# Vanlightly/vsr-tlaplus

Hardware: NVIDIA H100
Metric: unique states explored/sec (VSR.tla, shipped VSR.cfg constants) (higher is better)
Workload: dtype u32

## Files before the change

vsr-tlaplus_b200/csrc/vsr_actions.h:

```cpp
#ifndef VSR_ACTIONS_H
#define VSR_ACTIONS_H

#include <utility>

#include "vsr_layout.h"

namespace vsr {

struct RunCfg {
    int symmetry;
    int use_view;
    int invariant;
};

template <class L> struct Ops {
    static constexpr int R = L::R, V = L::V, K = L::K, O = L::O;

    static VSR_HD int primary(int v) { return (v - 1) % R; }
    static VSR_HD int oidx(int a, int b) { return b < a ? b : b - 1; }
    static VSR_HD int oinv(int a, int i) { return i < a ? i : i + 1; }

    template <int B, int N = 0, class W> static VSR_HD int loglen(const W& w, int row) {
        int n = 0;
        for (int i = 0; i < V; i++) {
            if (fget<B, L::OB, N>(w, row * V + i) == 0) break;
            n++;
        }
        return n;
    }
    template <int BD, int BS, class WD, class WS> static VSR_HD void logcopy(const WD& wd, int rowd, const WS& ws, int rows) {
        for (int i = 0; i < V; i++) fset<BD, L::OB>(wd, rowd * V + i, fget<BS, L::OB>(ws, rows * V + i));
    }
    template <int B, class W> static VSR_HD void logclear(const W& w, int row) {
        for (int i = 0; i < V; i++) fset<B, L::OB>(w, row * V + i, 0);
    }
    template <class W> static VSR_HD int popmask_svc(const W& w, int r) {
        int n = 0;
        for (int s = 0; s < R; s++) n += (int)VGET(L, SVC_MASK, w, r * R + s);
        return n;
    }
    template <class W> static VSR_HD int popmask_dvc(const W& w, int r) {
        int n = 0;
        for (int s = 0; s < R; s++) n += (int)VGET(L, DVC_MASK, w, r * R + s);
        return n;
    }
    template <class W> static VSR_HD void reset_recv(const W& w, int r) {
        for (int s = 0; s < R; s++) {
            VSET(L, SVC_MASK, w, r * R + s, 0);
            VSET(L, DVC_MASK, w, r * R + s, 0);
        }
        logclear<L::SELF_LOG_B>(w, r);
        VSET(L, SELF_LNV, w, r, 0);
        VSET(L, SELF_COMMIT, w, r, 0);
    }
    template <class W> static VSR_HD void reset_dvc_only(const W& w, int r) {
        for (int s = 0; s < R; s++) VSET(L, DVC_MASK, w, r * R + s, 0);
        logclear<L::SELF_LOG_B>(w, r);
        VSET(L, SELF_LNV, w, r, 0);
        VSET(L, SELF_COMMIT, w, r, 0);
    }
    template <class W> static VSR_HD void reset_sent(const W& w, int r) {
        VSET(L, SENT_DVC, w, r, 0);
        VSET(L, SENT_SV, w, r, 0);
    }
    static VSR_HD int svc_slot(int v, int s, int d) { return ((v - 2) * R + s) * O + oidx(s, d); }
    template <class W> static VSR_HD int broadcast_svc(const W& w, int v, int s) {
        for (int dp = 0; dp < O; dp++) {
            const int idx = ((v - 2) * R + s) * O + dp;
            if (VGET(L, SVC_ST, w, idx) != ST_ABSENT) return E_SLOT_OCCUPIED;
            VSET(L, SVC_ST, w, idx, ST_PENDING);
        }
        return 0;
    }
    template <class W> static VSR_HD int ncreated(const W& w) {
        int c = 0;
        for (int x = 0; x < V; x++) c += VGET(L, PR_VIEW, w, x) != 0;
        return c;
    }

    static constexpr int NGRP = 13;
    static VSR_HD constexpr int grp_begin(int g) {
        const int b[NGRP + 1] = {L::C_TIMER, L::C_HSVC, L::C_SDVC, L::C_HDVC, L::C_SSV, L::C_RSV, L::C_CREQ, L::C_RPREP,
                                 L::C_RPOK, L::C_EXEC, L::C_SGS, L::C_RGS, L::C_RNS, L::NCAND};
        return b[g];
    }
    template <bool APPLY, class S, class N> static VSR_HD int step(const RunCfg& run, const S& s, int cand, const N& n) {
        return cand < L::C_HSVC ? step_grp<APPLY, 0, S, N>(run, s, cand, n) : cand < L::C_SDVC ? step_grp<APPLY, 1, S, N>(run, s, cand, n)
             : cand < L::C_HDVC ? step_grp<APPLY, 2, S, N>(run, s, cand, n) : cand < L::C_SSV ? step_grp<APPLY, 3, S, N>(run, s, cand, n)
             : cand < L::C_RSV ? step_grp<APPLY, 4, S, N>(run, s, cand, n) : cand < L::C_CREQ ? step_grp<APPLY, 5, S, N>(run, s, cand, n)
             : cand < L::C_RPREP ? step_grp<APPLY, 6, S, N>(run, s, cand, n) : cand < L::C_RPOK ? step_grp<APPLY, 7, S, N>(run, s, cand, n)
             : cand < L::C_EXEC ? step_grp<APPLY, 8, S, N>(run, s, cand, n) : cand < L::C_SGS ? step_grp<APPLY, 9, S, N>(run, s, cand, n)
             : cand < L::C_RGS ? step_grp<APPLY, 10, S, N>(run, s, cand, n) : cand < L::C_RNS ? step_grp<APPLY, 11, S, N>(run, s, cand, n)
             : step_grp<APPLY, 12, S, N>(run, s, cand, n);
    }
    template <bool APPLY, int GRP, class S, class N> static VSR_HD int step_grp(const RunCfg& run, const S& s, int cand, const N& n) {
        if constexpr (APPLY) {
            for (int i = 0; i < L::NW; i++) wrw(n, i, rdw(s, i));
        }
        if constexpr (GRP == 0) {
            const int r = cand - L::C_TIMER;
            const int aux = (int)VGET(L, AUX_SVC, s, 0);
            if (!(aux < L::L)) return 0;
            const int v = (int)VGET(L, VIEWN, s, r);
// ... 260 lines not shown
            for (int p = 0; p < R; p++) q += (int)VGET(L, PEER, s, r * R + p) >= cn + 1;
            if (!(q >= R / 2)) return 0;
            if (!APPLY) return 1;
            VSET(L, COMMIT, n, r, cn + 1);
            VSET(L, CT_EXEC, n, r, 1);
            const int x = (int)VGET(L, LOG, s, r * V + cn);
            VSET(L, ACKED, n, x - 1, ACK_TRUE);
            return 1;
        }
        if constexpr (GRP == 10) {
            const int c = cand - L::C_SGS;
            const int j = c % O, dp = (c / O) % O, x = c / (O * O);
            const int pv = (int)VGET(L, PR_VIEW, s, x);
            if (pv == 0) return 0;
            if (VGET(L, PR_CONS, s, x * O + dp)) return 0;
            const int src = primary(pv);
            const int r = oinv(src, dp);
            const int rdest = oinv(r, j);
            const int vr = (int)VGET(L, VIEWN, s, r);
            if (primary(vr) == r) return 0;
            if (VGET(L, STATUS, s, r) != 0) return 0;
            if (!(pv > vr)) return 0;
            const int len = loglen<L::LOG_B, L::LOG_N>(s, r);
            if (!((int)VGET(L, PR_OP, s, x) > len + 1)) return 0;
            const int cn = (int)VGET(L, COMMIT, s, r);
            const int t = cn <= len ? cn : len;
            const int gi = (pv - 2) * O + oidx(src, r);
            if (VGET(L, GS_ST, s, gi) != ST_ABSENT) {
                if ((int)VGET(L, GS_T, s, gi) == t && (int)VGET(L, GS_DEST, s, gi) == rdest) return 0;
                return APPLY ? E_SLOT_OCCUPIED : 1;
            }
            if (!APPLY) return 1;
            if (popmask_svc(s, r) != 0 || popmask_dvc(s, r) != 0) return E_STALE_RECV;
            for (int i = t; i < V; i++) VSET(L, LOG, n, r * V + i, 0);
            VSET(L, VIEWN, n, r, pv);
            VSET(L, LNV, n, r, pv);
            VSET(L, GS_ST, n, gi, ST_PENDING);
            VSET(L, GS_T, n, gi, t);
            VSET(L, GS_DEST, n, gi, rdest);
            return 1;
        }
        if constexpr (GRP == 11) {
            const int gi = cand - L::C_RGS;
            if (VGET(L, GS_ST, s, gi) != ST_PENDING) return 0;
            const int v = gi / O + 2;
            const int r = (int)VGET(L, GS_DEST, s, gi);
            if ((int)VGET(L, VIEWN, s, r) != v) return 0;
            if (VGET(L, STATUS, s, r) != 0) return 0;
            const int t = (int)VGET(L, GS_T, s, gi);
            const int len = loglen<L::LOG_B, L::LOG_N>(s, r);
            if (!(len > t)) return 0;
            if (!APPLY) return 1;
            VSET(L, GS_ST, n, gi, ST_CONSUMED);
            if (VGET(L, NS_ST, s, gi) != ST_ABSENT) return E_SLOT_OCCUPIED;
            VSET(L, NS_ST, n, gi, ST_PENDING);
            for (int i = 0; i < V; i++) VSET(L, NS_LOG, n, gi * V + i, (i >= t && i < len) ? VGET(L, LOG, s, r * V + i) : 0);
            VSET(L, NS_COMMIT, n, gi, VGET(L, COMMIT, s, r));
            return 1;
        }
        if constexpr (GRP == 12) {
            const int gi = cand - L::C_RNS;
            if (VGET(L, NS_ST, s, gi) != ST_PENDING) return 0;
            const int v = gi / O + 2;
            const int r = oinv(primary(v), gi % O);
            if ((int)VGET(L, VIEWN, s, r) != v) return 0;
            if (VGET(L, STATUS, s, r) != 0) return 0;
            const int t = (int)VGET(L, GS_T, s, gi);
            if (loglen<L::LOG_B, L::LOG_N>(s, r) != t) return 0;
            if (!APPLY) return 1;
            for (int i = t; i < V; i++) VSET(L, LOG, n, r * V + i, VGET(L, NS_LOG, s, gi * V + i));
            VSET(L, NS_ST, n, gi, ST_CONSUMED);
            return 1;
        }
        return 0;
    }

    static VSR_HD constexpr int grp_size(int g) { return grp_begin(g + 1) - grp_begin(g); }
    static VSR_HD constexpr int grp_words(int g) { return (grp_size(g) + 31) / 32; }
    template <int G, class S, int... I>
    static VSR_HD void enabled_seq(const RunCfg& run, const S& s, uint32_t* mask, std::integer_sequence<int, I...>) {
        ((mask[I >> 5] |= (uint32_t)(step_grp<false, G>(run, s, grp_begin(G) + I, (uint32_t*)nullptr) > 0) << (I & 31)), ...);
    }
    template <int G, class S> static VSR_HD void enabled_group(const RunCfg& run, const S& s, uint32_t* mask) {
        enabled_seq<G>(run, s, mask, std::make_integer_sequence<int, grp_size(G)>());
    }

    template <int G> static VSR_HD int list_group(const RunCfg& run, const RegRow<L::NW>& st, uint32_t* out, int n) {
        uint32_t m[grp_words(G) > 0 ? grp_words(G) : 1] = {};
        enabled_group<G>(run, st, m);
        for (int i = 0; i < grp_size(G); i++)
            if ((m[i >> 5] >> (i & 31)) & 1u) out[n++] = (uint32_t)(grp_begin(G) + i);
        if constexpr (G + 1 < NGRP) return list_group<G + 1>(run, st, out, n);
        else return n;
    }
    static VSR_HD int enabled_list(const RunCfg& run, const uint32_t* w, uint32_t* out ) {
        RegRow<L::NW> st;
        for (int i = 0; i < L::NW; i++) st.w[i] = w[i];
        return list_group<0>(run, st, out, 0);
    }

    static VSR_HD int action_of(int cand) {
        return cand < L::C_HSVC ? 1 : cand < L::C_MSVC ? 2 : cand < L::C_SDVC ? 3 : cand < L::C_HDVC ? 4
             : cand < L::C_MDVC ? 5 : cand < L::C_SSV ? 6 : cand < L::C_RSV ? 7 : cand < L::C_CREQ ? 8
             : cand < L::C_RPREP ? 9 : cand < L::C_RPOK ? 10 : cand < L::C_EXEC ? 11 : cand < L::C_SGS ? 12
             : cand < L::C_RGS ? 13 : cand < L::C_RNS ? 14 : 15;
    }

    static VSR_HD void init(uint32_t* w) {
        for (int i = 0; i < L::NW; i++) w[i] = 0;
        for (int r = 0; r < R; r++) {
            VSET(L, VIEWN, w, r, 1);
            VSET(L, CT_EXEC, w, r, 1);
        }
    }

    template <class W> static VSR_HD int invariant(const RunCfg& run, const W& w) {
        if (run.invariant & 256) {
            for (int r = 0; r < R; r++)
                if ((int)VGET(L, COMMIT, w, r) == V) return 256;
        }
        if (!(run.invariant & 3)) return 0;
        for (int x = 0; x < V; x++) {
            if (VGET(L, ACKED, w, x) != ACK_TRUE) continue;
            int holders = 0;
            for (int r = 0; r < R; r++) {
                int has = 0;
                for (int i = 0; i < V; i++) has |= (int)VGET(L, LOG, w, r * V + i) == x + 1;
                holders += has;
            }
            if ((run.invariant & 1) && holders == 0) return 1;
            if ((run.invariant & 2) && holders < R / 2 + 1) return 2;
        }
        return 0;
    }

    template <class W> static VSR_HD bool all_same_view_normal(const RunCfg&, const W& w) {
        const uint32_t v0 = VGET(L, VIEWN, w, 0);
        for (int r = 0; r < R; r++)
            if (VGET(L, STATUS, w, r) != 0 || VGET(L, VIEWN, w, r) != v0) return false;
        return true;
    }
    template <class W> static VSR_HD bool some_commit(const W& w) {
        for (int r = 0; r < R; r++)
            if (VGET(L, COMMIT, w, r) >= 1) return true;
        return false;
    }
    template <class W> static VSR_HD bool live_pred(const RunCfg& run, const W& w, int live_hooks) {
        return (live_hooks & 1) ? some_commit(w) : all_same_view_normal(run, w);
    }

    template <class W> static VSR_HD uint32_t aux_key(const W& w) {
        uint32_t k = VGET(L, AUX_SVC, w, 0);
        k = k * 16u;
        for (int x = 0; x < V; x++) k = k * 3u + VGET(L, ACKED, w, x);
        return k;
    }

    static VSR_HD int literal_cand(const uint32_t* w, int cand) {
        if (cand < L::C_CREQ || cand >= L::C_RGS || (cand >= L::C_RPOK && cand < L::C_SGS)) return cand;
        if (cand < L::C_RPREP) {
            const int r = (cand - L::C_CREQ) / V;
            for (int x = 0; x < V; x++)
                if (VGET(L, PR_VIEW, w, x) == 0) return L::C_CREQ + r * V + x;
            return -1;
        }
        int order[V > 0 ? V : 1], nc = 0;
        for (int x = 0; x < V; x++)
// ... 177 lines not shown
```

vsr-tlaplus_b200/csrc/vsr_gpu.cu:

```cuda
#include <stddef.h>
#include <stdio.h>
#include <stdlib.h>
#include <string.h>

#include <algorithm>
#include <chrono>
#include <string>
#include <vector>

#include "vsr_engine.h"

namespace vsr {

const GpuOps* find_gpu_ops(int R, int V, int K) {
#define X(r, v, k) \
    if (R == r && V == v && K == k) return GpuThunks<Layout<r, v, k>>::get();
    VSR_FOR_EACH_CONFIG(X)
#undef X
    return nullptr;
}

}

using namespace vsr;
// ... 284 lines not shown
int vsr_engine_expand_part(VsrEngine* e, uint64_t first, uint64_t count) { return vsr_engine_step(e, first, count, 0, nullptr, nullptr); }

int vsr_engine_expand(VsrEngine* e) { return vsr_engine_step(e, 0, e->n_cur, 0, nullptr, nullptr); }

int vsr_engine_insert_records(VsrEngine* e, const void* dev_records, uint64_t n) {
    if (!e->level_open) {
        int rc = engine_reset_level(e);
        if (rc) return rc;
    }
    if (n == 0) return 0;
    const int rc = insert_records(e, dev_records, n);
    if (rc) return rc;
    CK(cudaEventSynchronize(e->ev1));
    float ms = 0;
    cudaEventElapsedTime(&ms, e->ev0, e->ev1);
    e->level_ms_acc += ms;
    e->level_ms_insert_acc += ms;
    return 0;
}

int vsr_engine_finish_level(VsrEngine* e, VsrLevelInfo* out) {
    LevelCounters lc;
    DevCounters& c = lc.c;
    const size_t ctr_bytes = e->cov ? sizeof lc : sizeof c;
    CK(cudaMemcpyAsync(&lc, e->ctr, ctr_bytes, cudaMemcpyDeviceToHost, e->stream));
    e->st.bytes_d2h += ctr_bytes;
    CK(cudaStreamSynchronize(e->stream));
    const uint64_t fcap_total = e->frontier_cap + e->frontier_host_cap;
    if (c.tie_count > 0 && c.tie_count <= e->tie_cap && !c.overflow && c.out_count <= fcap_total) {
        const size_t tb = (size_t)e->g->tie_bytes;
        std::vector<uint8_t> host(c.tie_count * tb);
        CK(cudaMemcpyAsync(host.data(), e->ties, host.size(), cudaMemcpyDeviceToHost, e->stream));
        CK(cudaStreamSynchronize(e->stream));
        std::vector<const uint8_t*> recs;
        for (uint64_t i = 0; i < c.tie_count; i++) recs.push_back(host.data() + i * tb);
        auto key = [](const uint8_t* r) { return (const TieRec*)r; };
        std::sort(recs.begin(), recs.end(), [&](const uint8_t* a, const uint8_t* b) {
            const TieRec *x = key(a), *y = key(b);
            if (x->fp != y->fp) return x->fp < y->fp;
            if (x->check != y->check) return x->check < y->check;
            if (x->auxkey != y->auxkey) return x->auxkey < y->auxkey;
            if (x->parent != y->parent) return x->parent < y->parent;
            return x->cand < y->cand;
        });
        std::vector<uint8_t> best;
        uint64_t nbest = 0;
        for (size_t i = 0; i < recs.size(); i++) {
            if (i && key(recs[i])->fp == key(recs[i - 1])->fp && key(recs[i])->check == key(recs[i - 1])->check) continue;
            best.insert(best.end(), recs[i], recs[i] + tb);
            nbest++;
        }
        CK(cudaMemcpyAsync(e->ties, best.data(), best.size(), cudaMemcpyHostToDevice, e->stream));
        static const unsigned long long ones = ~0ull;
        CK(cudaMemcpyAsync(&e->ctr->viol_id, &ones, 8, cudaMemcpyHostToDevice, e->stream));
        CK(cudaMemsetAsync(&e->ctr->viol_which, 0, sizeof(int), e->stream));
        ExpandParams p;
        fill_params(e, p);
        CK(e->g->launch_patch(p, e->ties, nbest, c.out_count, e->stream));
        e->st.kernel_launches++;
        CK(cudaMemcpyAsync(&lc, e->ctr, ctr_bytes, cudaMemcpyDeviceToHost, e->stream));
        CK(cudaStreamSynchronize(e->stream));
        e->st.bytes_d2h += host.size() + ctr_bytes;
        e->st.bytes_h2d += best.size();
    }
    VsrLevelInfo li;
    memset(&li, 0, sizeof li);
    li.new_states = c.out_count;
    li.generated = c.generated;
    li.frontier_in = e->n_cur;
    li.ties = c.ties;
    li.collisions = c.collisions;
    li.violation = c.viol_id != ~0ull;
    li.violation_id = c.viol_id;
    li.violation_mask = c.viol_which;
    li.deadlock = c.dead_id != ~0ull;
    li.deadlock_id = c.dead_id;
    li.error_code = c.error;
    li.overflow = c.overflow;
    li.ms = e->level_ms_acc;
    li.ms_insert = e->level_ms_insert_acc;
#ifdef VSR_EXP_ROUNDCLK
    {
        double all = 0;
        for (int i = 0; i < 5; i++) all += (double)c.roundclk[i];
        if (all > 0)
            fprintf(stderr, "roundclk rank %d depth %d  ms %.4f  warp-Gcycles %.4f  end_barrier %.4f  scan_barriers %.4f  batches %.4f  scan %.4f  other %.4f\n",
                    e->rank, e->level, e->level_ms_acc, all * 1e-9, c.roundclk[0] / all, c.roundclk[1] / all, c.roundclk[2] / all, c.roundclk[3] / all, c.roundclk[4] / all);
    }
#endif
    if (c.overflow) {
        snprintf(e->last_error, sizeof e->last_error, "capacity exceeded (%s): %llu new states this level, frontier capacity %llu",
                 c.overflow == 1 ? "frontier" : (c.overflow == 2 ? "tie list" : (c.overflow == 3 ? "send buffer" : "seen-set")), (unsigned long long)c.out_count,
                 (unsigned long long)fcap_total);
    }
    if (!li.overflow && e->st.distinct + c.out_count > e->table_cap - e->table_cap / 8) {
        li.overflow = 4;
        snprintf(e->last_error, sizeof e->last_error, "capacity exceeded (seen-set): %llu distinct states in %llu slots",
                 (unsigned long long)(e->st.distinct + c.out_count), (unsigned long long)e->table_cap);
    }
    const uint64_t n_new = c.out_count <= fcap_total ? c.out_count : fcap_total;
    e->st.generated += c.generated;
    e->st.distinct += n_new;
    e->st.h2_ties += c.ties;
    e->st.fp_collisions += c.collisions;
    e->st.probe_total += c.probes;
    e->st.seconds_kernels += e->level_ms_acc * 1e-3;
    if (c.error && !e->st.error_code) e->st.error_code = c.error;
    const int gen_level = e->level + 1;
    if (e->level >= 1 && e->level - 1 < VSR_MAX_LEVELS) {
        e->st.level_generated[e->level - 1] = c.generated;
        e->st.level_ms[e->level - 1] = e->level_ms_acc;
        e->st.levels_expanded = e->level;
    }
    if (n_new > 0 && gen_level - 1 < VSR_MAX_LEVELS) {
        e->st.level_sizes[gen_level - 1] = n_new;
        e->st.num_levels = gen_level;
    }
    if (e->cov && gen_level - 1 < VSR_MAX_LEVELS) {
        bool any = false;
        for (int a = 0; a < VSR_NUM_ACTIONS; a++) {
            const uint64_t g = lc.cover[a], d = lc.cover[VSR_NUM_ACTIONS + a];
            e->cov->level_generated[gen_level - 1][a] = g;
            e->cov->level_distinct[gen_level - 1][a] = d;
            e->cov->generated[a] += g;
            e->cov->distinct[a] += d;
            any |= g != 0;
        }
        if (any) e->cov->num_levels = gen_level;
    }
    if (li.violation && e->st.violation_level == 0) {
        e->st.violation_level = gen_level;
        e->st.violation_id = c.viol_id;
    }
    e->cur ^= 1;
    e->cur_base = e->next_base;
    e->n_cur = n_new;
    e->next_base += n_new;
    e->level = gen_level;
    e->level_open = false;
    if (e->live_index && !li.overflow) {
        const int rc = live_collect(e);
        if (rc == VSR_RC_TOO_LARGE) li.overflow = 5;
        else if (rc) return rc;
    }
    if (e->opts.collect_levels) {
        std::vector<uint8_t> host((size_t)n_new * e->g->bytes);
        if (n_new && vsr_engine_read_frontier(e, 0, n_new, host.data())) return VSR_RC_SYSTEM;
        e->collected.push_back(std::move(host));
    }
    if (out) *out = li;
    return 0;
}

uint64_t vsr_engine_frontier_size(const VsrEngine* e) { return e->n_cur; }

int vsr_engine_read_frontier(VsrEngine* e, uint64_t first, uint64_t n, void* host_out) {
    if (first + n > e->n_cur) return VSR_RC_ERROR;
    const uint64_t S = (uint64_t)e->g->bytes;
    const uint64_t in_dev = first < e->frontier_cap ? std::min(n, e->frontier_cap - first) : 0;
    if (in_dev) CK(cudaMemcpy(host_out, (const uint8_t*)e->frontier[e->cur] + first * S, in_dev * S, cudaMemcpyDeviceToHost));
    if (n > in_dev) memcpy((uint8_t*)host_out + in_dev * S, (const uint8_t*)e->frontier_host[e->cur] + (first + in_dev - e->frontier_cap) * S, (n - in_dev) * S);
    return 0;
}

int vsr_engine_trace_record(VsrEngine* e, uint64_t local_id, uint64_t* parent_out, uint32_t* cand_out) {
    if (!e->trace || local_id >= e->trace_cap) return VSR_RC_ERROR;
    uint64_t t = 0;
    CK(cudaMemcpy(&t, e->trace + local_id, 8, cudaMemcpyDeviceToHost));
    e->st.bytes_d2h += 8;
    *parent_out = (t >> 12) & GID_MASK;
// ... 230 lines not shown
```

vsr-tlaplus_b200/csrc/vsr_gpu.cuh:

```cuda
#ifndef VSR_GPU_CUH
#define VSR_GPU_CUH

#include <cuda_runtime.h>
#include <stdint.h>

#include "../../include/vsr_flat.h"
#include "vsr_actions.h"

namespace vsr {

struct DevCounters {
    unsigned long long out_count;
    unsigned long long generated;
    unsigned long long ties;
    unsigned long long collisions;
    unsigned long long probes;
    unsigned long long viol_id;
    unsigned long long dead_id;
    unsigned long long tie_count;
    int error;
    int overflow;
    int viol_which;
    int _pad;
    unsigned long long work_next;
    unsigned long long drain_next;
    unsigned int send_count[8];
#ifdef VSR_EXP_ROUNDCLK
    unsigned long long roundclk[5];
#endif
};
struct LevelCounters {
    DevCounters c;
    unsigned long long cover[2 * VSR_NUM_ACTIONS];
};
#ifdef VSR_EXP_ROUNDCLK
enum { CLK_END = 0, CLK_SCANBAR = 1, CLK_BATCH = 2, CLK_SCAN = 3, CLK_OTHER = 4 };
#endif

struct TieRec {
    uint64_t fp;
    uint64_t parent;
    uint32_t auxkey, cand, check, _pad;
};

struct RecHdr {
    uint64_t fp;
    uint64_t tm;
};
constexpr int MAX_WORLD = 8;


struct ExpandParams {
    const uint32_t* in;
    unsigned long long n_in;
    unsigned long long in_base;
    const uint32_t* in_hi;
    unsigned long long in_split;
    uint32_t* out;
    uint32_t* out_hi;
    unsigned long long out_split;
    unsigned long long out_cap;
    unsigned long long out_base;
    uint64_t* table;
    unsigned long long table_cap;
    uint64_t* trace;
    unsigned long long trace_cap;
    DevCounters* ctr;
    uint8_t* ties;
    unsigned long long tie_cap;
    const uint64_t* fp_tab;
    RunCfg run;
    int level;
    int check_deadlock;
    int rank, world, owner_shift;
    uint8_t* push[MAX_WORLD];
    unsigned long long push_cap;
    const uint8_t* drain[MAX_WORLD];
    unsigned int drain_n[MAX_WORLD];
    unsigned long long drain_total;
    unsigned long long* cover;
};


__device__ __forceinline__ void cas128(uint64_t* p, uint64_t s0, uint64_t s1, uint64_t& o0, uint64_t& o1) {
    asm volatile(
        "{\n\t.reg .b128 cmp, swp, old;\n\tmov.b128 cmp, {%2, %3};\n\tmov.b128 swp, {%4, %5};\n\t"
        "atom.global.relaxed.gpu.cas.b128 old, [%6], cmp, swp;\n\tmov.b128 {%0, %1}, old;\n\t}"
        : "=l"(o0), "=l"(o1)
        : "l"(0ull), "l"(0ull), "l"(s0), "l"(s1), "l"(p)
        : "memory");
}
__device__ __forceinline__ void ld128_cg(const uint64_t* p, uint64_t& a, uint64_t& b) {
    asm volatile("ld.global.cg.v2.u64 {%0, %1}, [%2];" : "=l"(a), "=l"(b) : "l"(p) : "memory");
}
__device__ __forceinline__ uint64_t mix64(uint64_t x) {
    x ^= x >> 30; x *= 0xbf58476d1ce4e5b9ULL;
    x ^= x >> 27; x *= 0x94d049bb133111ebULL;
    x ^= x >> 31;
    return x;
}
template <class L, bool USE_VIEW, class W> VSR_HD uint32_t check_hash_t(const W& w) {
    constexpr int full = L::VIEW_BITS >> 5, rem = L::VIEW_BITS & 31;
    constexpr int nw = USE_VIEW ? (full + (rem ? 1 : 0)) : L::NW;
    uint32_t h = 0x9747b28cu;
VSR_UNROLL
    for (int i = 0; i < nw; i++) {
        uint32_t k = rdw(w, i);
        if (USE_VIEW && i == full) k &= (1u << rem) - 1u;
        h ^= k;
        h = ((h << 13) | (h >> 19)) * 5u + 0xe6546b64u;
    }
    h ^= h >> 16; h *= 0x85ebca6bu; h ^= h >> 13; h *= 0xc2b2ae35u; h ^= h >> 16;
    return h;
}
template <class L, class W> VSR_HD uint32_t check_hash(const W& w, bool use_view) {
    return use_view ? check_hash_t<L, true>(w) : check_hash_t<L, false>(w);
}

enum { INS_NEW = 0, INS_DUP = 1, INS_TIE = 2, INS_FULL = 3 };

constexpr unsigned long long GID_MASK = (1ull << 44) - 1ull, ROOT_GID = GID_MASK;
__host__ __device__ __forceinline__ uint64_t make_gid(int rank, unsigned long long local_id) { return ((uint64_t)rank << 40) | local_id; }
__host__ __device__ __forceinline__ uint64_t make_trec(uint64_t parent_gid, uint32_t cand) { return (parent_gid << 12) | (cand & 0xFFFu); }

__device__ __forceinline__ uint64_t make_meta(int level, uint32_t auxkey, uint32_t check) {
    return ((uint64_t)(uint32_t)level << 56) | ((uint64_t)(auxkey & 0xFFFFFFu) << 32) | check;
}

#ifndef VSR_BUCKET
#define VSR_BUCKET 2
#endif
struct Probe { uint64_t e[2 * VSR_BUCKET]; };
__device__ __forceinline__ void ld256_cg(const uint64_t* p, uint64_t& a, uint64_t& b, uint64_t& c, uint64_t& d) {
    asm volatile("ld.global.cg.v2.u64 {%0, %1}, [%4];\n\tld.global.cg.v2.u64 {%2, %3}, [%4+16];"
                 : "=l"(a), "=l"(b), "=l"(c), "=l"(d) : "l"(p) : "memory");
}
__device__ __forceinline__ unsigned long long table_home(unsigned long long cap, uint64_t fp) {
    return __umul64hi(fp * 0x9E3779B97F4A7C15ULL, cap / VSR_BUCKET) * VSR_BUCKET;
}
__device__ __forceinline__ void probe_load(const uint64_t* table, unsigned long long h, Probe& p) {
#if VSR_BUCKET == 1
    ld128_cg(table + 2 * h, p.e[0], p.e[1]);
#elif VSR_BUCKET == 2
    ld128_cg(table + 2 * h, p.e[0], p.e[1]);
#elif VSR_BUCKET == 4
    ld256_cg(table + 2 * h, p.e[0], p.e[1], p.e[2], p.e[3]);
    ld256_cg(table + 2 * h + 4, p.e[4], p.e[5], p.e[6], p.e[7]);
#else
#error "VSR_BUCKET must be 1, 2 or 4"
#endif
}
__device__ __forceinline__ int table_insert_from(uint64_t* table, unsigned long long cap, unsigned long long h, Probe p, uint64_t fp, uint64_t meta,
                                                 unsigned& probes, unsigned& collisions) {
    for (unsigned tries = 0;; tries++) {
        if (tries > (1u << 16)) return INS_FULL;
        probes++;
VSR_UNROLL
        for (int j = 0; j < VSR_BUCKET; j++) {
            uint64_t e0, e1;
            if (VSR_BUCKET == 2 && j == 1) {
                ld128_cg(table + 2 * (h + 1), e0, e1);
            } else {
                e0 = p.e[2 * j];
                e1 = p.e[2 * j + 1];
            }
            if (e0 == 0) {
                cas128(table + 2 * (h + j), fp, meta, e0, e1);
                if (e0 == 0 && e1 == 0) return INS_NEW;
            }
            for (int again = 0; e1 == 0 && again < 64; again++) ld128_cg(table + 2 * (h + j), e0, e1);
            if (e0 == fp) {
                if ((uint32_t)e1 == (uint32_t)meta) {
                    const bool same_level = (e1 >> 56) == (meta >> 56);
                    const bool same_aux = ((e1 >> 32) & 0xFFFFFF) == ((meta >> 32) & 0xFFFFFF);
// ... 19 lines not shown
    asm volatile("fence.proxy.async.shared::cta;" ::: "memory");
    const uint32_t s = (uint32_t)__cvta_generic_to_shared(ssrc);
    asm volatile("cp.async.bulk.global.shared::cta.bulk_group [%0], [%1], %2;" ::"l"(gdst), "r"(s), "r"(bytes) : "memory");
    asm volatile("cp.async.bulk.commit_group;" ::: "memory");
    asm volatile("cp.async.bulk.wait_group.read 0;" ::: "memory");
}

template <int NW> __device__ __forceinline__ uint32_t* out_state(const ExpandParams& P, unsigned long long i) {
    return i < P.out_split ? P.out + i * NW : P.out_hi + (i - P.out_split) * NW;
}


#ifdef VSR_QPS
constexpr int QPS = VSR_QPS;
#else
constexpr int QPS = 10;
#endif

template <class L, int ROWS> struct WarpStage {
    alignas(16) uint32_t stage[ROWS * L::NW + 32];
    unsigned long long tstage[ROWS];
    int sn;
};
template <class L, int WARPS, int PASSES> struct BlockSmemT {
    typedef WarpStage<L, PASSES == 2 ? 32 : 64> Stage;
    static constexpr int NS = WARPS * 32;
    static constexpr int NR = PASSES * NS;
    static constexpr int NG = 13;
    uint64_t fp_tab[8 * 256];
    uint32_t par[NR * (L::NW + 1)];
    static constexpr int QCAP = QPS * NS;
    uint16_t pool[PASSES * QCAP];
    int qcount[PASSES][NG];
    int take;
    unsigned long long round_first;
    Stage w[WARPS];
};
template <class L> struct ExpandCfg {
    static constexpr size_t SMEM_ONE = 227 * 1024 - 512, SMEM_TWO = 113 * 1024;
    static constexpr int max_grp() { int m = 0; for (int g = 0; g < Ops<L>::NGRP; g++) m = Ops<L>::grp_size(g) > m ? Ops<L>::grp_size(g) : m; return m; }
    template <int W> static constexpr int pick_one() {
        if constexpr (W < 18) return 0;
        else if constexpr (sizeof(BlockSmemT<L, W, 1>) <= SMEM_ONE) return W;
        else return pick_one<W - 2>();
    }
    static constexpr int W2 = sizeof(BlockSmemT<L, 16, 1>) <= SMEM_TWO ? 16 : (sizeof(BlockSmemT<L, 12, 1>) <= SMEM_TWO ? 12 : 8);
    static constexpr int W1 = max_grp() < 64 ? pick_one<32>() : 0;
#ifdef VSR_FORCE_WARPS
    static constexpr int WARPS = VSR_FORCE_WARPS;
#else
    static constexpr int WARPS = W1 >= 2 * W2 - 4 ? W1 : W2;
#endif
    static constexpr int BLOCKS = WARPS > 16 ? 1 : 2;
#ifdef VSR_ROUND_PASSES
    static constexpr int PASSES = VSR_ROUND_PASSES;
#else
    static constexpr int PASSES = BLOCKS == 1 && sizeof(BlockSmemT<L, WARPS, 2>) <= SMEM_ONE ? 2 : 1;
#endif
    typedef BlockSmemT<L, WARPS, PASSES> Smem;
};

template <class L, bool MULTI, bool COVER = false> struct Expander {
    typedef Ops<L> O_;
    typedef typename ExpandCfg<L>::Smem Smem;
    typedef typename Smem::Stage Stage;
    static constexpr int WARPS = ExpandCfg<L>::WARPS, NS = Smem::NS, PASSES = ExpandCfg<L>::PASSES;
    static constexpr int SROWS = PASSES == 2 ? 32 : 64;
    const ExpandParams& P;
    Smem& B;
    Stage& S;
    const int lane, warp, tid;
    const uint32_t* mine = nullptr;
    bool have = false;
    int pass = 0;
    __device__ __forceinline__ int pass_i() const { return PASSES == 1 ? 0 : pass; }

    __device__ Expander(const ExpandParams& p, Smem& b) : P(p), B(b), S(b.w[threadIdx.x >> 5]), lane(threadIdx.x & 31), warp(threadIdx.x >> 5), tid(threadIdx.x) {
#ifdef VSR_EXP_ROUNDCLK
        clk_t = clock64();
#endif
    }

#ifdef VSR_EXP_ROUNDCLK
    unsigned long long clk_t = 0, clk[5] = {};
    __device__ __forceinline__ void clk_mark(int i) {
        const unsigned long long t = clock64();
        clk[i] += t - clk_t;
        clk_t = t;
    }
#define VSR_CLK(X, i) (X).clk_mark(CLK_##i)
#else
#define VSR_CLK(X, i) ((void)0)
#endif

    static __device__ __noinline__ void flush(const ExpandParams& P, Stage& S, int lane, int n) {
        const int sn = SROWS == 32 ? n : S.sn;
        unsigned long long base = 0;
        if (lane == 0) base = atomicAdd(&P.ctr->out_count, (unsigned long long)n);
        base = __shfl_sync(0xffffffffu, base, 0);
        if (lane < n) {
            const unsigned long long t = S.tstage[lane];
            if (t >> 63) {
                atomicMin(&P.ctr->viol_id, P.out_base + base + lane);
                S.tstage[lane] = t & ~(1ull << 63);
            }
        }
        __syncwarp();
        if (base + n > P.out_cap) {
            if (lane == 0) atomicExch(&P.ctr->overflow, 1);
        } else {
            if (lane == 0) {
                if (base + n <= P.out_split) bulk_store(P.out + base * L::NW, S.stage, (uint32_t)(n * L::BYTES));
                else if (base >= P.out_split) bulk_store(P.out_hi + (base - P.out_split) * L::NW, S.stage, (uint32_t)(n * L::BYTES));
                else {
                    const int n1 = (int)(P.out_split - base);
                    bulk_store(P.out + base * L::NW, S.stage, (uint32_t)(n1 * L::BYTES));
                    bulk_store(P.out_hi, S.stage + n1 * L::NW, (uint32_t)((n - n1) * L::BYTES));
                }
            }
            if (P.trace && lane < n && P.out_base + base + lane < P.trace_cap) P.trace[P.out_base + base + lane] = S.tstage[lane];
        }
        __syncwarp();
        const int rest = sn - n;
        for (int i0 = 0; i0 < rest * L::NW; i0 += 32) {
            const int i = i0 + lane;
            uint32_t v = 0;
            if (i < rest * L::NW) v = S.stage[n * L::NW + i];
            __syncwarp();
            if (i < rest * L::NW) S.stage[i] = v;
        }
        unsigned long long t = 0;
        if (lane < rest) t = S.tstage[n + lane];
        __syncwarp();
        if (lane < rest) S.tstage[lane] = t;
        if (lane == 0) S.sn = rest;
        __syncwarp();
    }

    typedef uint32_t* Row;
    static constexpr int gcd32(int a) { int g = 32; while (a % g) g >>= 1; return g; }
    static constexpr int SKEW_P = 32 / gcd32(L::NW);
    static __device__ __forceinline__ Row scratch(Stage& S, int lane) { return &S.stage[(SROWS - 32 + lane) * L::NW + lane / SKEW_P]; }

    static __device__ __forceinline__ void push_records(const ExpandParams& P, Stage& S, int lane, const RegRow<L::NW>& v, int send_to, uint64_t fp,
                                                        uint64_t tm) {
        const unsigned senders = __ballot_sync(0xffffffffu, send_to >= 0);
        if (!senders) return;
        constexpr int RB = L::BYTES + (int)sizeof(RecHdr), RW = RB / 4;
        constexpr int CAPREC = (32 * L::BYTES) / RB;
        static_assert(CAPREC >= 16, "two passes must cover a batch");
        int off = 0, cnt = 0, rnk = 0;
        unsigned mymask = 0;
        for (int d = 0; d < P.world; d++) {
            const unsigned m = __ballot_sync(0xffffffffu, send_to == d);
            if (send_to > d) off += __popc(m);
            if (send_to == d) { mymask = m; cnt = __popc(m); rnk = __popc(m & ((1u << lane) - 1u)); }
        }
        unsigned base = 0;
        if (send_to >= 0 && rnk == 0) base = atomicAdd(&P.ctr->send_count[send_to], (unsigned)cnt);
        base = __shfl_sync(0xffffffffu, base, mymask ? __ffs(mymask) - 1 : 0);
        const bool fits = send_to >= 0 && (unsigned long long)base + (unsigned)cnt <= P.push_cap;
        if (send_to >= 0 && !fits && rnk == 0) atomicExch(&P.ctr->overflow, 3);
        const int pos = off + rnk, total = __popc(senders);
        uint32_t* sbuf = &S.stage[(SROWS - 32) * L::NW];
        for (int lo = 0; lo < total; lo += CAPREC) {
            const int hi = lo + CAPREC < total ? lo + CAPREC : total;
            if (send_to >= 0 && pos >= lo && pos < hi) {
// ... 183 lines not shown
                v.w[4 * q] = x.x; v.w[4 * q + 1] = x.y; v.w[4 * q + 2] = x.z; v.w[4 * q + 3] = x.w;
            }
            chk = check_hash<L>(v, P.run.use_view != 0);
            auxkey = O_::aux_key(v);
        }
        tally(commit(P, S, lane, v, d.have, d.fp, chk, auxkey, d.home, d.first, d.tm & ((1ull << 56) - 1ull), (unsigned)((d.tm >> 56) & 0xFu)));
    }
    __device__ void drain() {
        const unsigned long long nchunks = drain_chunks();
        if (dchunk == ~0ull) dchunk = __shfl_sync(0xffffffffu, drain_claim(), 0);
        while (dchunk < nchunks) {
            const unsigned long long nx = drain_claim();
            const DrainPre d = drain_begin(dchunk);
            drain_end(d);
            dchunk = __shfl_sync(0xffffffffu, nx, 0);
        }
    }

    static constexpr int NG = O_::NGRP;
    static __host__ __device__ constexpr int moff(int g) { int o = 0; for (int h = 0; h < g; h++) o += O_::grp_words(h); return o; }
    static constexpr int MW = moff(NG);
    static constexpr int PW = (NG + 1) / 2;
    static __host__ __device__ constexpr int max_grp() { int m = 0; for (int g = 0; g < NG; g++) m = O_::grp_size(g) > m ? O_::grp_size(g) : m; return m; }
    static constexpr int TBITS = NS <= 512 ? 9 : 10;
    static_assert(NS <= (1 << TBITS) && max_grp() < (1 << (16 - TBITS)), "pool item does not fit 16 bits");
    static_assert(max_grp() * NS < 65536, "16-bit packed counters");

    template <int G> __device__ __forceinline__ void guards(const RegRow<L::NW>& st, uint32_t* m, uint32_t* pc) {
        O_::template enabled_group<G>(P.run, st, m + moff(G));
        uint32_t c = 0;
        VSR_UNROLL
        for (int k = 0; k < O_::grp_words(G); k++) c += (uint32_t)__popc(m[moff(G) + k]);
        pc[G >> 1] += c << (16 * (G & 1));
        if constexpr (G + 1 < NG) guards<G + 1>(st, m, pc);
    }
    template <int G, bool FAST> __device__ __forceinline__ void push(uint32_t* m, const uint32_t* ex, const uint32_t* wb, int st) {
        int pos = st + (int)((wb[G >> 1] >> (16 * (G & 1))) & 0xFFFFu) + (int)((ex[G >> 1] >> (16 * (G & 1))) & 0xFFFFu);
        VSR_UNROLL
        for (int k = 0; k < O_::grp_words(G); k++) {
            uint32_t mm = m[moff(G) + k], left = 0;
            while (mm) {
                const int bit = __ffs(mm) - 1;
                mm &= mm - 1;
                if (FAST || pos < Smem::QCAP) B.pool[pass_i() * Smem::QCAP + pos] = (uint16_t)(tid | ((k * 32 + bit) << TBITS));
                else left |= 1u << bit;
                pos++;
            }
            if (!FAST) m[moff(G) + k] = left;
        }
        if constexpr (G + 1 < NG) {
            const int q = B.qcount[pass_i()][G];
            const int nst = FAST ? st + q : (st + q < Smem::QCAP ? st + q : Smem::QCAP);
            push<G + 1, FAST>(m, ex, wb, nst);
        }
    }
    template <int G> __device__ __forceinline__ void leftovers(uint32_t* m) {
        VSR_UNROLL
        for (int k = 0; k < O_::grp_words(G); k++) {
            while (__any_sync(0xffffffffu, m[moff(G) + k] != 0)) {
                const bool inl = m[moff(G) + k] != 0;
                int cand = 0;
                if (inl) {
                    const int bit = __ffs(m[moff(G) + k]) - 1;
                    m[moff(G) + k] &= m[moff(G) + k] - 1;
                    cand = O_::grp_begin(G) + k * 32 + bit;
                }
                tally(apply<G>(P, B, S, lane, mine, cand, pass_i() * NS + tid, inl));
            }
        }
        if constexpr (G + 1 < NG) leftovers<G + 1>(m);
    }
    __device__ __forceinline__ void scan_all() {
        uint32_t m[MW], pc[PW];
        VSR_UNROLL
        for (int i = 0; i < MW; i++) m[i] = 0;
        VSR_UNROLL
        for (int i = 0; i < PW; i++) pc[i] = 0;
        if (have) {
            RegRow<L::NW> st;
            VSR_UNROLL
            for (int i = 0; i < L::NW; i++) st.w[i] = mine[i];
            guards<0>(st, m, pc);
        }
        uint32_t ex[PW], wb[PW];
        VSR_UNROLL
        for (int i = 0; i < PW; i++) ex[i] = pc[i];
        VSR_UNROLL
        for (int o = 1; o < 32; o <<= 1) {
            VSR_UNROLL
            for (int i = 0; i < PW; i++) {
                const uint32_t t = __shfl_up_sync(0xffffffffu, ex[i], o);
                if (lane >= o) ex[i] += t;
            }
        }
        uint32_t mytot = 0, anyc = 0;
        VSR_UNROLL
        for (int g = 0; g < NG; g++) {
            const uint32_t t = (__shfl_sync(0xffffffffu, ex[g >> 1], 31) >> (16 * (g & 1))) & 0xFFFFu;
            if (lane == g) mytot = t;
        }
        VSR_UNROLL
        for (int i = 0; i < PW; i++) { anyc |= pc[i]; ex[i] -= pc[i]; }
        uint32_t mybase = 0;
        if (lane < NG && mytot) mybase = (uint32_t)atomicAdd(&B.qcount[pass_i()][lane], (int)mytot);
        VSR_UNROLL
        for (int i = 0; i < PW; i++) wb[i] = 0;
        VSR_UNROLL
        for (int g = 0; g < NG; g++) wb[g >> 1] |= (__shfl_sync(0xffffffffu, mybase, g) & 0xFFFFu) << (16 * (g & 1));
        if (P.check_deadlock && have && !anyc) atomicMin(&P.ctr->dead_id, P.in_base + B.round_first + pass_i() * NS + tid);
        VSR_CLK(*this, SCAN);
        __syncthreads();
        VSR_CLK(*this, SCANBAR);
#ifndef VSR_EXP_NO_PUSHFAST
        int all = 0;
        VSR_UNROLL
        for (int g = 0; g < NG; g++) all += B.qcount[pass_i()][g];
        if (all <= Smem::QCAP) {
            push<0, true>(m, ex, wb, 0);
            return;
        }
#endif
        push<0, false>(m, ex, wb, 0);
        uint32_t rest = 0;
        VSR_UNROLL
        for (int i = 0; i < MW; i++) rest |= m[i];
        if (__any_sync(0xffffffffu, rest != 0)) leftovers<0>(m);
    }
    template <int G> static __device__ __noinline__ unsigned long long apply(const ExpandParams& P, Smem& B, Stage& S, int lane,
                                                                             const uint32_t* parent, int cand, int si, bool act) {
        const Row n = scratch(S, lane);
        int mult = 0;
        if (act) mult = O_::template step_grp<true, G>(P.run, parent, cand, n);
        return emit(P, B, S, lane, n, mult, cand, si, act);
    }
    template <int G> static __device__ __forceinline__ unsigned long long batch(const ExpandParams& P, Smem& B, Stage& S, int lane, int b,
                                                                                int k) {
        const bool act = lane < k;
        int cand = 0, si = 0;
        if (act) {
            const unsigned item = B.pool[b + lane];
            si = (PASSES == 1 ? 0 : b / Smem::QCAP) * NS + (int)(item & ((1 << TBITS) - 1));
            cand = O_::grp_begin(G) + (int)(item >> TBITS);
        }
        return apply<G>(P, B, S, lane, &B.par[si * (L::NW + 1)], cand, si, act);
    }
    unsigned long long acc_gen = 0, acc_probes = 0;
    __device__ __forceinline__ void tally(unsigned long long r) {
        acc_gen += (unsigned)r;
        acc_probes += r >> 32;
    }

    __device__ void run_round(unsigned long long first, int count) {
        const uint32_t* src = P.in + first * L::NW;
        if (first + count <= P.in_split) {
            for (int i = tid; i < count * L::NW; i += NS) B.par[(i / L::NW) * (L::NW + 1) + (i % L::NW)] = __ldg(src + i);
        } else {
            for (int i = tid; i < count * L::NW; i += NS) {
                const unsigned long long st = first + i / L::NW;
                const uint32_t* row = st < P.in_split ? P.in + st * L::NW : P.in_hi + (st - P.in_split) * L::NW;
                B.par[(i / L::NW) * (L::NW + 1) + (i % L::NW)] = __ldg(row + i % L::NW);
            }
        }
        if (tid < PASSES * Smem::NG) (&B.qcount[0][0])[tid] = 0;
        if (tid == 0) { B.round_first = first; B.take = 0; }
        VSR_CLK(*this, SCAN);
        __syncthreads();
        VSR_CLK(*this, SCANBAR);
#pragma unroll 1
        for (pass = 0; pass < PASSES; pass++) {
            have = pass_i() * NS + tid < count;
            mine = &B.par[(have ? pass_i() * NS + tid : 0) * (L::NW + 1)];
            scan_all();
        }
        VSR_CLK(*this, SCAN);
        __syncthreads();
        VSR_CLK(*this, SCANBAR);
        static_assert(PASSES * Smem::NG <= 32, "one lane per segment");
        const int sp = lane / Smem::NG;
        const int q = lane < PASSES * Smem::NG ? (&B.qcount[0][0])[lane] : 0;
        int inc = q;
        VSR_UNROLL
        for (int o = 1; o < 32; o <<= 1) {
            const int t = __shfl_up_sync(0xffffffffu, inc, o);
            if (lane >= o) inc += t;
        }
        const int before = __shfl_sync(0xffffffffu, inc, sp * Smem::NG - 1 + (sp == 0));
        if (sp > 0) inc -= before;
        const int seg_st = sp * Smem::QCAP + (inc - q < Smem::QCAP ? inc - q : Smem::QCAP), seg_en = sp * Smem::QCAP + (inc < Smem::QCAP ? inc : Smem::QCAP);
        const int nb = (seg_en - seg_st + 31) >> 5;
        int binc = nb;
        VSR_UNROLL
        for (int o = 1; o < 32; o <<= 1) {
            const int t = __shfl_up_sync(0xffffffffu, binc, o);
            if (lane >= o) binc += t;
        }
        const int total = __shfl_sync(0xffffffffu, binc, 31);
        for (;;) {
            int t = 0;
            if (lane == 0) t = atomicAdd(&B.take, 1);
            t = __shfl_sync(0xffffffffu, t, 0);
            if (t >= total) break;
            const int s = __popc(__ballot_sync(0xffffffffu, lane < PASSES * Smem::NG && binc <= t));
            const int st = __shfl_sync(0xffffffffu, seg_st, s), en = __shfl_sync(0xffffffffu, seg_en, s);
            const int b = st + (t - __shfl_sync(0xffffffffu, binc - nb, s)) * 32;
            const int k = en - b < 32 ? en - b : 32;
            unsigned long long r;
            switch (s % Smem::NG) {
            case 0: r = batch<0>(P, B, S, lane, b, k); break;   case 1: r = batch<1>(P, B, S, lane, b, k); break;
            case 2: r = batch<2>(P, B, S, lane, b, k); break;   case 3: r = batch<3>(P, B, S, lane, b, k); break;
            case 4: r = batch<4>(P, B, S, lane, b, k); break;   case 5: r = batch<5>(P, B, S, lane, b, k); break;
            case 6: r = batch<6>(P, B, S, lane, b, k); break;   case 7: r = batch<7>(P, B, S, lane, b, k); break;
            case 8: r = batch<8>(P, B, S, lane, b, k); break;   case 9: r = batch<9>(P, B, S, lane, b, k); break;
            case 10: r = batch<10>(P, B, S, lane, b, k); break; case 11: r = batch<11>(P, B, S, lane, b, k); break;
            default: r = batch<12>(P, B, S, lane, b, k); break;
            }
            tally(r);
            VSR_CLK(*this, BATCH);
        }
        VSR_CLK(*this, BATCH);
    }

    __device__ void finish() {
        while (S.sn > 0) flush(P, S, lane, S.sn < 32 ? S.sn : 32);
#ifdef VSR_EXP_ROUNDCLK
        clk_mark(CLK_OTHER);
        VSR_UNROLL
        for (int i = 0; i < 5; i++)
            if (lane == 0) atomicAdd(&P.ctr->roundclk[i], clk[i]);
#endif
        for (int o = 16; o; o >>= 1) {
            acc_gen += __shfl_xor_sync(0xffffffffu, acc_gen, o);
            acc_probes += __shfl_xor_sync(0xffffffffu, acc_probes, o);
        }
        if (lane == 0) {
            atomicAdd(&P.ctr->generated, acc_gen);
            atomicAdd(&P.ctr->probes, acc_probes);
        }
        if constexpr (COVER && COVER_SHARED) {
            __syncthreads();
            const unsigned long long* tab = cover_table(P);
            if (tid < NCOV && tab[tid]) atomicAdd(&P.cover[tid], tab[tid]);
        }
    }
};

template <class L, bool MULTI, bool COVER = false> __global__ void __launch_bounds__(ExpandCfg<L>::WARPS * 32, ExpandCfg<L>::BLOCKS) expand_kernel(const __grid_constant__ ExpandParams P) {
    extern __shared__ __align__(128) unsigned char smem_raw[];
    typedef typename ExpandCfg<L>::Smem Smem;
    Smem& B = *reinterpret_cast<Smem*>(smem_raw);
    for (int i = threadIdx.x; i < 8 * 256; i += blockDim.x) B.fp_tab[i] = P.fp_tab[i];
    __shared__ unsigned long long next_round;
    Expander<L, MULTI, COVER> X(P, B);
    if ((threadIdx.x & 31) == 0) B.w[threadIdx.x >> 5].sn = 0;
    if constexpr (COVER && Expander<L, MULTI, COVER>::COVER_SHARED) {
        if (threadIdx.x < Expander<L, MULTI, COVER>::NCOV) Expander<L, MULTI, COVER>::cover_table(P)[threadIdx.x] = 0;
    }
    const unsigned long long nrounds = (P.n_in + Smem::NR - 1) / Smem::NR;
    if (threadIdx.x == 0) next_round = atomicAdd(&P.ctr->work_next, 1ull);
    VSR_CLK(X, OTHER);
    for (;;) {
        __syncthreads();
        const unsigned long long c = next_round;
        __syncthreads();
        VSR_CLK(X, END);
        if (c >= nrounds) break;
        if (threadIdx.x == 0) {
            next_round = atomicAdd(&P.ctr->work_next, 1ull);
            const unsigned long long nx = next_round;
            if (nx < nrounds && (nx + 1) * Smem::NR <= P.in_split) {
                const unsigned long long nfirst = nx * Smem::NR;
                const unsigned long long ncount = (P.n_in - nfirst) < (unsigned long long)Smem::NR ? (P.n_in - nfirst) : Smem::NR;
                asm volatile("cp.async.bulk.prefetch.L2.global [%0], %1;" ::"l"(P.in + nfirst * L::NW), "r"((uint32_t)(ncount * L::BYTES)) : "memory");
            }
        }
        const unsigned long long first = c * Smem::NR;
        const int count = (int)((P.n_in - first) < (unsigned long long)Smem::NR ? (P.n_in - first) : Smem::NR);
        X.run_round(first, count);
    }
    if (MULTI && P.drain_total) X.drain();
    X.finish();
}

template <class L> __global__ void patch_ties_kernel(const ExpandParams P, const uint8_t* ties, unsigned long long ntie, unsigned long long n_out) {
    const unsigned long long i = (unsigned long long)blockIdx.x * blockDim.x + threadIdx.x;
    if (i >= n_out) return;
    uint32_t w[L::NW];
    uint32_t* st = out_state<L::NW>(P, i);
    for (int j = 0; j < L::NW; j++) w[j] = st[j];
    uint64_t fp = fp64_view8<L>(P.fp_tab, w, P.run.use_view != 0);
    if (fp == 0) fp = 1;
    const uint32_t chk = check_hash<L>(w, P.run.use_view != 0);
    const size_t stride = sizeof(TieRec) + L::BYTES;
    unsigned long long lo = 0, hi = ntie;
    while (lo < hi) {
        const unsigned long long mid = (lo + hi) / 2;
        if (((const TieRec*)(ties + mid * stride))->fp < fp) lo = mid + 1; else hi = mid;
    }
    for (; lo < ntie; lo++) {
        const TieRec* t = (const TieRec*)(ties + lo * stride);
        if (t->fp != fp) break;
        if (t->check != chk) continue;
        if (t->auxkey < Ops<L>::aux_key(w)) {
            const uint32_t* tw = (const uint32_t*)((const uint8_t*)t + sizeof(TieRec));
            for (int j = 0; j < L::NW; j++) { w[j] = tw[j]; st[j] = tw[j]; }
            if (P.trace && P.out_base + i < P.trace_cap) {
                if (P.cover) {
                    const uint64_t was = P.trace[P.out_base + i];
                    const int a0 = (was >> 12) == ROOT_GID ? (int)VSR_ACT_INIT : Ops<L>::action_of((int)(was & 0xFFFu));
                    const int a1 = t->parent == ROOT_GID ? (int)VSR_ACT_INIT : Ops<L>::action_of((int)(t->cand & 0xFFFu));
                    if (a0 != a1) {
// ... 221 lines not shown
```

Baseline: 2.969 billion.

## Vectorize guard scans over slot bitmasks and load parent rows with cp.async

Replaces per-candidate guard evaluation for several action groups with word-level bitmask computation. Pending message slots are masked against per-class enable predicates evaluated once per class, and the even bits are compacted into the enabled mask. Groups 11 and 12 now iterate only over pending slots. Parent-state loads into shared memory use cp.async instead of register round-trips, and the clock-profiling buckets are split for finer scan timing. The risk is heavy template code whose slot-to-candidate mapping must exactly match the original per-candidate guards.

After: 3.046 billion (median of 6 runs). +2.6%, better.

```diff
diff --git a/vsr-tlaplus_b200/csrc/vsr_actions.h b/vsr-tlaplus_b200/csrc/vsr_actions.h
--- a/vsr-tlaplus_b200/csrc/vsr_actions.h
+++ b/vsr-tlaplus_b200/csrc/vsr_actions.h
@@ -16,9 +16,9 @@
 template <class L> struct Ops {
     static constexpr int R = L::R, V = L::V, K = L::K, O = L::O;
 
-    static VSR_HD int primary(int v) { return (v - 1) % R; }
-    static VSR_HD int oidx(int a, int b) { return b < a ? b : b - 1; }
-    static VSR_HD int oinv(int a, int i) { return i < a ? i : i + 1; }
+    static VSR_HD constexpr int primary(int v) { return (v - 1) % R; }
+    static VSR_HD constexpr int oidx(int a, int b) { return b < a ? b : b - 1; }
+    static VSR_HD constexpr int oinv(int a, int i) { return i < a ? i : i + 1; }
 
     template <int B, int N = 0, class W> static VSR_HD int loglen(const W& w, int row) {
         int n = 0;
@@ -445,7 +445,112 @@
         ((mask[I >> 5] |= (uint32_t)(step_grp<false, G>(run, s, grp_begin(G) + I, (uint32_t*)nullptr) > 0) << (I & 31)), ...);
     }
     template <int G, class S> static VSR_HD void enabled_group(const RunCfg& run, const S& s, uint32_t* mask) {
+#ifndef VSR_EXP_SCAN_PERCAND
+        if constexpr (G == 1 || G == 3 || G == 5 || G == 8) {
+            enabled_slots<G>(run, s, mask);
+            return;
+        } else if constexpr (G == 11 || G == 12) {
+            enabled_pending<G>(run, s, mask);
+            return;
+        }
+#endif
         enabled_seq<G>(run, s, mask, std::make_integer_sequence<int, grp_size(G)>());
+    }
+
+    static VSR_HD constexpr int slot_cls(int g, int i) {
+        return g == 1 ? (i / (O * R)) * R + oinv((i / O) % R, i % O)
+             : g == 3 ? i / O
+             : g == 5 ? (i / O) * R + oinv(primary(i / O + 2), i % O)
+             : i;
+    }
+    static VSR_HD constexpr int slot_base(int g) { return g == 1 ? L::SVC_ST_B : g == 3 ? L::DVC_ST_B : g == 5 ? L::SV_ST_B : g == 8 ? L::POK_ST_B : g == 11 ? L::GS_ST_B : L::NS_ST_B; }
+    static VSR_HD constexpr int slot_n(int g) { return g == 1 ? L::NSVC : g == 3 ? L::NDVC : g == 5 ? L::NSV : g == 8 ? L::NPOK : L::NGS; }
+    static VSR_HD constexpr int slot_ncls(int g) { return g == 1 ? L::NV2 * R : g == 3 ? L::NV2 : g == 5 ? L::NV2 * R : slot_n(g); }
+    static VSR_HD constexpr int slot_outs(int g) { return g == 1 || g == 3 ? 2 : 1; }
+    static VSR_HD constexpr uint32_t cls_mask(int g, int k, int c) {
+        uint32_t m = 0;
+        for (int i = 0; i < slot_n(g); i++) {
+            const int p = slot_base(g) + 2 * i;
+            if ((p >> 5) == k && (c < 0 || slot_cls(g, i) == c)) m |= 1u << (p & 31);
+        }
+        return m;
+    }
+    template <int G, int K, int C> static constexpr uint32_t CLS_MASK = cls_mask(G, K, C);
+    template <int G, int OUT, int C, class S> static VSR_HD bool cls_on(const S& s) {
+        if constexpr (G == 1) {
+            constexpr int v = C / R + 2, r = C % R;
+            const int vr = (int)VGET(L, VIEWN, s, r);
+            if constexpr (OUT == 0) return v > vr;
+            else return v == vr && VGET(L, STATUS, s, r) == 1;
+        } else if constexpr (G == 3) {
+            constexpr int v = C + 2, r = primary(v);
+            const int vr = (int)VGET(L, VIEWN, s, r);
+            return OUT == 0 ? v > vr : v == vr;
+        } else if constexpr (G == 5) {
+            constexpr int v = C / R + 2, r = C % R;
+            return v >= (int)VGET(L, VIEWN, s, r);
+        } else {
+            constexpr int sp = C % O, nn = (C / O) % V + 1, v = C / (O * V) + 1;
+            constexpr int r = primary(v), src = oinv(r, sp);
+            return v == (int)VGET(L, VIEWN, s, r) && VGET(L, STATUS, s, r) == 0 && nn > (int)VGET(L, PEER, s, r * R + src);
+        }
+    }
+    template <int G, int OUT, int K, class S, int... C> static VSR_HD uint32_t sel_word(const S& s, std::integer_sequence<int, C...>) {
+        uint32_t m = 0;
+        ((m |= (CLS_MASK<G, K, C> != 0u && cls_on<G, OUT, C>(s)) ? CLS_MASK<G, K, C> : 0u), ...);
+        return m;
+    }
+    static VSR_HD uint32_t gather_even(uint32_t x) {
+        x &= 0x55555555u;
+        x = (x | (x >> 1)) & 0x33333333u;
+        x = (x | (x >> 2)) & 0x0F0F0F0Fu;
+        x = (x | (x >> 4)) & 0x00FF00FFu;
+        return (x | (x >> 8)) & 0x0000FFFFu;
+    }
+    template <int G, int SH> static VSR_HD void put_bits(uint32_t* mask, uint32_t c) {
+        if constexpr (SH < 0) {
+            put_bits<G, 0>(mask, c >> -SH);
+        } else {
+            mask[SH >> 5] |= c << (SH & 31);
+            if constexpr ((SH & 31) > 16 && (SH >> 5) + 1 < grp_words(G)) mask[(SH >> 5) + 1] |= c >> (32 - (SH & 31));
+        }
+    }
+    template <int G, int K, class S> static VSR_HD uint32_t pending_word(const S& s) {
+        const uint32_t w = rdw(s, K);
+        return w & ~(w >> 1) & CLS_MASK<G, K, -1>;
+    }
+    template <int G, int K, class S> static VSR_HD void slots_word(const S& s, uint32_t* mask) {
+        constexpr int B = slot_base(G), N = slot_n(G);
+        const uint32_t pend = pending_word<G, K>(s);
+        constexpr int D = 16 * K - B / 2;
+        put_bits<G, D>(mask, gather_even(pend & sel_word<G, 0, K>(s, std::make_integer_sequence<int, slot_ncls(G)>())));
+        if constexpr (slot_outs(G) == 2) put_bits<G, D + N>(mask, gather_even(pend & sel_word<G, 1, K>(s, std::make_integer_sequence<int, slot_ncls(G)>())));
+        if constexpr (K + 1 <= ((B + 2 * N - 1) >> 5)) slots_word<G, K + 1>(s, mask);
+    }
+    template <int G, class S> static VSR_HD void enabled_slots(const RunCfg&, const S& s, uint32_t* mask) {
+        static_assert(slot_base(G) % 2 == 0, "2-bit slots start at even bits");
+        if constexpr (slot_n(G) > 0) slots_word<G, (slot_base(G) >> 5)>(s, mask);
+    }
+    template <int G, int K, class S> static VSR_HD void pending_loop(const RunCfg& run, const S& s, uint32_t* mask) {
+        constexpr int B = slot_base(G);
+        uint32_t pend = pending_word<G, K>(s);
+        while (pend) {
+#if defined(__CUDA_ARCH__)
+            const int bit = __ffs(pend) - 1;
+#else
+            const int bit = __builtin_ctz(pend);
+#endif
+            pend &= pend - 1;
+            const int i = (32 * K + bit - B) >> 1;
+            if (step_grp<false, G>(run, s, grp_begin(G) + i, (uint32_t*)nullptr) > 0) {
+                VSR_UNROLL
+                for (int q = 0; q < grp_words(G); q++) mask[q] |= (i >> 5) == q ? 1u << (i & 31) : 0u;
+            }
+        }
+        if constexpr (K + 1 <= ((B + 2 * slot_n(G) - 1) >> 5)) pending_loop<G, K + 1>(run, s, mask);
+    }
+    template <int G, class S> static VSR_HD void enabled_pending(const RunCfg& run, const S& s, uint32_t* mask) {
+        if constexpr (slot_n(G) > 0) pending_loop<G, (slot_base(G) >> 5)>(run, s, mask);
     }
 
     template <int G> static VSR_HD int list_group(const RunCfg& run, const RegRow<L::NW>& st, uint32_t* out, int n) {
diff --git a/vsr-tlaplus_b200/csrc/vsr_gpu.cu b/vsr-tlaplus_b200/csrc/vsr_gpu.cu
--- a/vsr-tlaplus_b200/csrc/vsr_gpu.cu
+++ b/vsr-tlaplus_b200/csrc/vsr_gpu.cu
@@ -390,10 +390,13 @@
 #ifdef VSR_EXP_ROUNDCLK
     {
         double all = 0;
-        for (int i = 0; i < 5; i++) all += (double)c.roundclk[i];
+        for (int i = 0; i < CLK_N; i++) all += (double)c.roundclk[i];
         if (all > 0)
-            fprintf(stderr, "roundclk rank %d depth %d  ms %.4f  warp-Gcycles %.4f  end_barrier %.4f  scan_barriers %.4f  batches %.4f  scan %.4f  other %.4f\n",
-                    e->rank, e->level, e->level_ms_acc, all * 1e-9, c.roundclk[0] / all, c.roundclk[1] / all, c.roundclk[2] / all, c.roundclk[3] / all, c.roundclk[4] / all);
+            fprintf(stderr, "roundclk rank %d depth %d  ms %.4f  warp-Gcycles %.4f  end_barrier %.4f  scan_barriers %.4f  batches %.4f  scan %.4f  other %.4f"
+                            "  scan_load %.4f  scan_guards %.4f  scan_reserve %.4f  scan_layout %.4f\n",
+                    e->rank, e->level, e->level_ms_acc, all * 1e-9, c.roundclk[CLK_END] / all, c.roundclk[CLK_SCANBAR] / all, c.roundclk[CLK_BATCH] / all,
+                    (c.roundclk[CLK_SCAN] + c.roundclk[CLK_GUARD] + c.roundclk[CLK_RESERVE] + c.roundclk[CLK_LAYOUT]) / all, c.roundclk[CLK_OTHER] / all,
+                    c.roundclk[CLK_SCAN] / all, c.roundclk[CLK_GUARD] / all, c.roundclk[CLK_RESERVE] / all, c.roundclk[CLK_LAYOUT] / all);
     }
 #endif
     if (c.overflow) {
diff --git a/vsr-tlaplus_b200/csrc/vsr_gpu.cuh b/vsr-tlaplus_b200/csrc/vsr_gpu.cuh
--- a/vsr-tlaplus_b200/csrc/vsr_gpu.cuh
+++ b/vsr-tlaplus_b200/csrc/vsr_gpu.cuh
@@ -26,7 +26,7 @@
     unsigned long long drain_next;
     unsigned int send_count[8];
 #ifdef VSR_EXP_ROUNDCLK
-    unsigned long long roundclk[5];
+    unsigned long long roundclk[8];
 #endif
 };
 struct LevelCounters {
@@ -34,7 +34,7 @@
     unsigned long long cover[2 * VSR_NUM_ACTIONS];
 };
 #ifdef VSR_EXP_ROUNDCLK
-enum { CLK_END = 0, CLK_SCANBAR = 1, CLK_BATCH = 2, CLK_SCAN = 3, CLK_OTHER = 4 };
+enum { CLK_END = 0, CLK_SCANBAR = 1, CLK_BATCH = 2, CLK_SCAN = 3, CLK_OTHER = 4, CLK_GUARD = 5, CLK_RESERVE = 6, CLK_LAYOUT = 7, CLK_N = 8 };
 #endif
 
 struct TieRec {
@@ -90,6 +90,10 @@
         : "l"(0ull), "l"(0ull), "l"(s0), "l"(s1), "l"(p)
         : "memory");
 }
+__device__ __forceinline__ void cp_async4(uint32_t* sdst, const uint32_t* gsrc) {
+    asm volatile("cp.async.ca.shared.global [%0], [%1], 4;" ::"r"((uint32_t)__cvta_generic_to_shared(sdst)), "l"(gsrc) : "memory");
+}
+__device__ __forceinline__ void cp_async_wait_all() { asm volatile("cp.async.wait_all;" ::: "memory"); }
 __device__ __forceinline__ void ld128_cg(const uint64_t* p, uint64_t& a, uint64_t& b) {
     asm volatile("ld.global.cg.v2.u64 {%0, %1}, [%2];" : "=l"(a), "=l"(b) : "l"(p) : "memory");
 }
@@ -275,7 +279,7 @@
     }
 
 #ifdef VSR_EXP_ROUNDCLK
-    unsigned long long clk_t = 0, clk[5] = {};
+    unsigned long long clk_t = 0, clk[CLK_N] = {};
     __device__ __forceinline__ void clk_mark(int i) {
         const unsigned long long t = clock64();
         clk[i] += t - clk_t;
@@ -625,6 +629,7 @@
             for (int i = 0; i < L::NW; i++) st.w[i] = mine[i];
             guards<0>(st, m, pc);
         }
+        VSR_CLK(*this, GUARD);
         uint32_t ex[PW], wb[PW];
         VSR_UNROLL
         for (int i = 0; i < PW; i++) ex[i] = pc[i];
@@ -651,7 +656,7 @@
         VSR_UNROLL
         for (int g = 0; g < NG; g++) wb[g >> 1] |= (__shfl_sync(0xffffffffu, mybase, g) & 0xFFFFu) << (16 * (g & 1));
         if (P.check_deadlock && have && !anyc) atomicMin(&P.ctr->dead_id, P.in_base + B.round_first + pass_i() * NS + tid);
-        VSR_CLK(*this, SCAN);
+        VSR_CLK(*this, RESERVE);
         __syncthreads();
         VSR_CLK(*this, SCANBAR);
 #ifndef VSR_EXP_NO_PUSHFAST
@@ -660,6 +665,7 @@
         for (int g = 0; g < NG; g++) all += B.qcount[pass_i()][g];
         if (all <= Smem::QCAP) {
             push<0, true>(m, ex, wb, 0);
+            VSR_CLK(*this, LAYOUT);
             return;
         }
 #endif
@@ -668,6 +674,7 @@
         VSR_UNROLL
         for (int i = 0; i < MW; i++) rest |= m[i];
         if (__any_sync(0xffffffffu, rest != 0)) leftovers<0>(m);
+        VSR_CLK(*this, LAYOUT);
     }
     template <int G> static __device__ __noinline__ unsigned long long apply(const ExpandParams& P, Smem& B, Stage& S, int lane,
                                                                              const uint32_t* parent, int cand, int si, bool act) {
@@ -696,7 +703,8 @@
     __device__ void run_round(unsigned long long first, int count) {
         const uint32_t* src = P.in + first * L::NW;
         if (first + count <= P.in_split) {
-            for (int i = tid; i < count * L::NW; i += NS) B.par[(i / L::NW) * (L::NW + 1) + (i % L::NW)] = __ldg(src + i);
+            for (int i = tid; i < count * L::NW; i += NS) cp_async4(&B.par[(i / L::NW) * (L::NW + 1) + (i % L::NW)], src + i);
+            cp_async_wait_all();
         } else {
             for (int i = tid; i < count * L::NW; i += NS) {
                 const unsigned long long st = first + i / L::NW;
@@ -768,7 +776,7 @@
 #ifdef VSR_EXP_ROUNDCLK
         clk_mark(CLK_OTHER);
         VSR_UNROLL
-        for (int i = 0; i < 5; i++)
+        for (int i = 0; i < CLK_N; i++)
             if (lane == 0) atomicAdd(&P.ctr->roundclk[i], clk[i]);
 #endif
         for (int o = 16; o; o >>= 1) {
```
